# DanielBrosch/SDPSymmetryReduction.jl

Measured on AMD Instinct MI355X. Metric: N x N SDP reductions/sec (admissible_subspace+blockDiagonalize) at N=4096, higher is better.
Workload: dtype int8 square (int32 acc) + f64 eigen

## Files before the change

### sdpsymmetryreduction.jl_amd/csrc/kernels_blockdiag.hip

```cpp
#include <cstdlib>
#include <type_traits>
#include "host_internal.h"
#include "kernel_util.h"

namespace sdpsr {

typedef double v4d __attribute__((ext_vector_type(4)));

__global__ void block_norms_kernel(int64_t n, int64_t ld, const double* __restrict__ M,
                                   const int32_t* __restrict__ space_of, int neig,
                                   unsigned long long* __restrict__ norms) {
    const int64_t len = n * n;
    const int64_t stride = (int64_t)gridDim.x * blockDim.x;
    for (int64_t e0 = (int64_t)blockIdx.x * blockDim.x; e0 < len; e0 += stride) {
        const int64_t e = e0 + threadIdx.x;
        bool valid = e < len;
        int64_t j = valid ? e / n : 0, i = valid ? e - j * n : 0;
        int bi = space_of[i], bj = space_of[j];
        unsigned long long v = valid ? (unsigned long long)__double_as_longlong(fabs(M[i + j * ld])) : 0ull;
        int key = bi * neig + bj;
        int prev_key = __shfl_up(key, 1, 64);
        bool head = ((threadIdx.x & 63) == 0) || prev_key != key;
#pragma unroll
        for (int o = 1; o < 64; o <<= 1) {
// ... 708 lines not shown
    const double* Ti = T + (int64_t)i * n * S1;
    double a0 = 0, a1 = 0;
    if (o < S) {
        const int ca = colA[o], cb = colB[o];
        int r = g;
        for (; r + 64 < n; r += 128) {
            const double qa0 = Qrm[(int64_t)r * S1 + ca], qb0 = Qrm[(int64_t)r * S1 + cb];
            const double ta0 = Ti[(int64_t)r * S1 + ca], tb0 = Ti[(int64_t)r * S1 + cb];
            const double qa1 = Qrm[(int64_t)(r + 64) * S1 + ca], qb1 = Qrm[(int64_t)(r + 64) * S1 + cb];
            const double ta1 = Ti[(int64_t)(r + 64) * S1 + ca], tb1 = Ti[(int64_t)(r + 64) * S1 + cb];
            a0 = fma(qa0, tb0, a0);
            a0 = fma(qb0, ta0, a0);
            a1 = fma(qa1, tb1, a1);
            a1 = fma(qb1, ta1, a1);
        }
        for (; r < n; r += 64) {
            a0 = fma(Qrm[(int64_t)r * S1 + ca], Ti[(int64_t)r * S1 + cb], a0);
            a0 = fma(Qrm[(int64_t)r * S1 + cb], Ti[(int64_t)r * S1 + ca], a0);
        }
    }
    red[threadIdx.x] = a0 + a1;
    __syncthreads();
    if (threadIdx.x < 4 && o < S) {
        double v = 0;
        for (int gg = 0; gg < 64; ++gg) v += red[gg * 4 + threadIdx.x];
        out[(int64_t)i * S + o] = (fabs(v) < atol) ? 0.0 : v;
    }
}

bool basis_image_two_stage_fits(int64_t n, int64_t d, int64_t S1) {
    return n <= 65535 && (2 * (d + 2) * 4 + n * 2) <= 60 * 1024 && d * n * S1 * 8 <= ((int64_t)4 << 30);
}

__global__ void __launch_bounds__(256)
class_sums_small_d_kernel(int n, int d, uint32_t first, int tstride, const uint32_t* __restrict__ L, const double* __restrict__ x,
                          double* __restrict__ out, int64_t ldo) {
    extern __shared__ __attribute__((aligned(16))) double cs_smem[];
    double* sx = cs_smem;
    const int lane = threadIdx.x & 63, wave = threadIdx.x >> 6;
    double* acc = cs_smem + n + (size_t)wave * 64 * tstride;
    double* mine = acc + (size_t)lane * tstride;
    for (int c = threadIdx.x; c < n; c += 256) sx[c] = x[c];
    __syncthreads();
    const int rows_per_round = gridDim.x * 4;
    const int bpr = (n + 511) / 512;
    const int my_rows = (n - blockIdx.x * 4 + rows_per_round - 1) / rows_per_round;
    const int total = my_rows * bpr;
    auto fetch = [&](int bq, uint32_t (&lab)[8]) {
        const int rr = bq / bpr, bb = bq - rr * bpr;
        const int r = blockIdx.x * 4 + rr * rows_per_round + wave;
        const uint32_t* col = L + (int64_t)((bq < total && r < n) ? r : 0) * n;
#pragma unroll
        for (int u = 0; u < 8; ++u) {
            const int c = bb * 512 + u * 64 + lane;
            lab[u] = col[c < n ? c : n - 1];
        }
    };
    auto process = [&](int bq, const uint32_t (&lab)[8]) {
        if (bq >= total) return;
        const int rr = bq / bpr, bb = bq - rr * bpr;
        if (bb == 0)
            for (int i = 0; i <= d; ++i) mine[i] = 0.0;
        double vv[8];
#pragma unroll
        for (int u = 0; u < 8; ++u) {
            const int c = bb * 512 + u * 64 + lane;
            vv[u] = c < n ? sx[c] : 0.0;
        }
#pragma unroll
        for (int u = 0; u < 8; ++u) atomicAdd(&mine[window_label(lab[u], first, (uint32_t)d)], vv[u]);
        if (bb == bpr - 1) {
            const int r = blockIdx.x * 4 + rr * rows_per_round + wave;
            __syncthreads();
            if (r < n)
                for (int i = 1 + lane; i <= d; i += 64) {
                    double t = 0;
                    for (int l2 = 0; l2 < 64; ++l2) t += acc[(size_t)l2 * tstride + i];
                    out[(int64_t)(i - 1) * ldo + r] = t;
                }
            __syncthreads();
        }
    };
    uint32_t qa[8], qb[8], qc[8], qd[8];
    fetch(0, qa);
    fetch(1, qb);
    fetch(2, qc);
#pragma unroll 1
    for (int bq = 0; bq < total; bq += 4) {
        fetch(bq + 3, qd);
        process(bq, qa);
        fetch(bq + 4, qa);
        process(bq + 1, qb);
        fetch(bq + 5, qb);
        process(bq + 2, qc);
        fetch(bq + 6, qc);
        process(bq + 3, qd);
    }
}

__device__ __forceinline__ double bi_weight(uint64_t key, int k) {
    return 0.5 + (double)(sdpsr_fmix64(key + 0x9E3779B97F4A7C15ULL * (uint64_t)(k + 1)) >> 11) * (1.0 / 9007199254740992.0);
}

__global__ void bi_signed_sums_kernel(int n, int S1, const double* __restrict__ Qrm, uint64_t key, double2* __restrict__ X, uint32_t* flag) {
    const int r = blockIdx.x * blockDim.x + threadIdx.x;
    if (blockIdx.x == 0)
        for (int k = threadIdx.x; k <= S1; k += blockDim.x) flag[k] = 0u;
    if (r >= n) return;
    double a = 0, b = 0;
    for (int k = 0; k < S1; ++k) {
        const double q = Qrm[(int64_t)r * S1 + k];
        a += q;
        b = fma(bi_weight(key, k), q, b);
    }
    X[r] = make_double2(a, b);
}

__global__ void bi_pair_vector_kernel(int n, int S1, const double* __restrict__ Qrm, int k1, int k2, double2* __restrict__ X) {
    const int r = blockIdx.x * blockDim.x + threadIdx.x;
    if (r < n) X[r] = make_double2(Qrm[(int64_t)r * S1 + k1], Qrm[(int64_t)r * S1 + k2]);
}

__global__ void __launch_bounds__(256)
bi_contract_pair_kernel(int n, int S1, const double* __restrict__ Qrm, const double2* __restrict__ Y, int k1, int k2, double atol,
                        double* __restrict__ out) {
    __shared__ double red[2][256];
    const int i = blockIdx.x;
    const double2* Yi = Y + (int64_t)i * n;
    double a0 = 0, a1 = 0;
// ... 25 lines not shown
    const int bpr = (n + 511) / 512;
    const int my_rows = (n - (int)blockIdx.x * W + rows_per_round - 1) / rows_per_round;
    const int total = my_rows * bpr;
    auto fetch = [&](int bq, uint32_t (&lab)[8], double2 (&xv)[8]) {
        const int rr = bq / bpr, bb = bq - rr * bpr;
        const int r = blockIdx.x * W + rr * rows_per_round + wave;
        const uint32_t* col = L + (int64_t)((bq < total && r < n) ? r : 0) * n;
#pragma unroll
        for (int u = 0; u < 8; ++u) {
            const int c = bb * 512 + u * 64 + lane;
            const int cc = c < n ? c : n - 1;
            lab[u] = col[cc];
            xv[u] = X[cc];
        }
    };
    auto process = [&](int bq, const uint32_t (&lab)[8], const double2 (&xv)[8]) {
        if (bq >= total) return;
        const int rr = bq / bpr, bb = bq - rr * bpr;
        if (bb == 0)
            for (int i = 0; i <= d; ++i) mine[i] = make_double2(0.0, 0.0);
#pragma unroll
        for (int u = 0; u < 8; ++u) {
            const int c = bb * 512 + u * 64 + lane;
            if (c < n) {
                const uint32_t l = WIN ? window_label(lab[u], first, (uint32_t)d) : lab[u];
                double2 t = mine[l];
                t.x += xv[u].x;
                t.y += xv[u].y;
                mine[l] = t;
            }
        }
        if (bb == bpr - 1) {
            const int r = blockIdx.x * W + rr * rows_per_round + wave;
            __syncthreads();
            if (r < n)
                for (int i = 1 + lane; i <= d; i += 64) {
                    double tx = 0, ty = 0;
                    for (int l2 = 0; l2 < 64; ++l2) {
                        const double2 v = acc[(size_t)l2 * tstride + i];
                        tx += v.x;
                        ty += v.y;
                    }
                    out[(int64_t)(i - 1) * n + r] = make_double2(tx, ty);
                }
            __syncthreads();
        }
    };
    uint32_t la[8], lb[8], lc[8];
    double2 xa[8], xb[8], xc[8];
    fetch(0, la, xa);
    fetch(1, lb, xb);
#pragma unroll 1
    for (int bq = 0; bq < total; bq += 3) {
        fetch(bq + 2, lc, xc);
        process(bq, la, xa);
        fetch(bq + 3, la, xa);
        process(bq + 1, lb, xb);
        fetch(bq + 4, lb, xb);
        process(bq + 2, lc, xc);
    }
}

__global__ void __launch_bounds__(256)
bi_contract_check_kernel(int n, int S1, const double* __restrict__ Qrm, const double2* __restrict__ Y, uint64_t key, double atol,
                         double tol, double* __restrict__ out, uint32_t* __restrict__ flag) {
    __shared__ double red[2][256];
    const int i = blockIdx.x;
    const int k = blockIdx.y * 4 + (threadIdx.x & 3);
    const int g = threadIdx.x >> 2;
    const double2* Yi = Y + (int64_t)i * n;
    double a0 = 0, a1 = 0;
    if (k < S1)
        for (int r0 = g; r0 < n; r0 += 64 * 8) {
            double q[8];
            double2 y[8];
#pragma unroll
            for (int x = 0; x < 8; ++x) {
                const int r = r0 + 64 * x;
                const int rc = r < n ? r : g;
                q[x] = r < n ? Qrm[(int64_t)rc * S1 + k] : 0.0;
                y[x] = Yi[rc];
            }
#pragma unroll
            for (int x = 0; x < 8; ++x) {
                a0 = fma(q[x], y[x].x, a0);
                a1 = fma(q[x], y[x].y, a1);
            }
        }
    red[0][threadIdx.x] = a0;
    red[1][threadIdx.x] = a1;
    __syncthreads();
    if (threadIdx.x < 4 && k < S1) {
        double v0 = 0, v1 = 0;
        for (int gg = 0; gg < 64; ++gg) {
            v0 += red[0][gg * 4 + threadIdx.x];
            v1 += red[1][gg * 4 + threadIdx.x];
        }
        if (!(fabs(v0 - v1 / bi_weight(key, k)) <= tol)) {
            if (atomicExch(&flag[1 + k], 1u) == 0u) atomicAdd(&flag[0], 1u);
        }
        out[(int64_t)i * S1 + k] = (fabs(v0) < atol) ? 0.0 : v0;
    }
}

static void launch_class_sums2(hipStream_t s, int W, int g, size_t lds, int64_t n, int64_t d, uint32_t first, bool plain, int tstride, const uint32_t* L,
                               const double2* X, double2* Y) {
    if (plain && first == 1u) {
        if (W == 4) class_sums2_kernel<4, false><<<g, 256, lds, s>>>((int)n, (int)d, first, tstride, L, X, Y);
        else if (W == 2) class_sums2_kernel<2, false><<<g, 128, lds, s>>>((int)n, (int)d, first, tstride, L, X, Y);
        else class_sums2_kernel<1, false><<<g, 64, lds, s>>>((int)n, (int)d, first, tstride, L, X, Y);
    } else {
        if (W == 4) class_sums2_kernel<4, true><<<g, 256, lds, s>>>((int)n, (int)d, first, tstride, L, X, Y);
        else if (W == 2) class_sums2_kernel<2, true><<<g, 128, lds, s>>>((int)n, (int)d, first, tstride, L, X, Y);
        else class_sums2_kernel<1, true><<<g, 64, lds, s>>>((int)n, (int)d, first, tstride, L, X, Y);
    }
}

int launch_class_sums_pair(hipStream_t s, int64_t n, int64_t d, uint32_t first, bool plain, const uint32_t* L, const double* X, double* Y) {
    const int tstride = (int)((d + 1) | 1);
    const size_t per_wave = (size_t)64 * tstride * sizeof(double2);
    int W = 4;
    while (W > 1 && per_wave * W > 150 * 1024) W >>= 1;
    if (per_wave * W > 150 * 1024 || n < 1 || n > 0x7FFFFFFF / 2) return 0;
    int g = (int)((n + W - 1) / W);
    if (g > 256) g = 256;
    launch_class_sums2(s, W, g, per_wave * W, n, d, first, plain, tstride, L, reinterpret_cast<const double2*>(X), reinterpret_cast<double2*>(Y));
    return W;
}

size_t basis_image_commutative_workspace_doubles(int64_t n, int64_t d) { return (size_t)2 * n * (d + 1); }
bool launch_basis_image_commutative(hipStream_t s, int64_t n, int64_t d, uint32_t first, int64_t S1, const uint32_t* L, const double* Qrm, uint64_t key,
                                    double atol, double tol, double* ws, double* out, uint32_t* flag, bool plain) {
    const int tstride = (int)((d + 1) | 1);
    const size_t per_wave = (size_t)64 * tstride * sizeof(double2);
    int W = 4;
    while (W > 1 && per_wave * W > 150 * 1024) W >>= 1;
    if (per_wave * W > 150 * 1024 || n < 1 || n > 0x7FFFFFFF / 2) return false;
    double2* X = reinterpret_cast<double2*>(ws);
    double2* Y = X + n;
// ... 173 lines not shown
    const int tstride = (int)((d + 1) | 1);
    const size_t per_wave = (size_t)64 * tstride * sizeof(double2);
    int W = 4;
    while (W > 1 && per_wave * W > 150 * 1024) W >>= 1;
    if (per_wave * W > 150 * 1024 || n < 1 || n > 0x7FFFFFFF / 2 || nblocks < 1 || nblocks > 65535) return false;
    double2* X0 = reinterpret_cast<double2*>(ws);
    double2* X1 = X0 + n;
    double2* Y0 = X1 + n;
    double2* Y1 = Y0 + (size_t)d * n;
    double* ginv = reinterpret_cast<double*>(Y1 + (size_t)d * n);
    if ((size_t)S1 * BIB_T * 8 > 48 * 1024) return false;
    bib_vectors_kernel<<<(unsigned)((n + 255) / 256), 256, (size_t)S1 * BIB_T * 8, s>>>((int)n, (int)S1, nblocks, blk_col, blk_size, key, only, Qrm, X0, X1, only < 0 ? flag : nullptr, ginv);
    int g = (int)((n + W - 1) / W);
    if (g > 256) g = 256;
    const size_t lds = per_wave * W;
    for (int pass = 0; pass < 2; ++pass) {
        const double2* X = pass ? X1 : X0;
        double2* Y = pass ? Y1 : Y0;
        launch_class_sums2(s, W, g, lds, n, d, first, plain, tstride, L, X, Y);
    }
    dim3 gc((unsigned)d, only >= 0 ? 1u : (unsigned)nblocks);
    bib_contract_kernel<<<gc, 256, 0, s>>>((int)n, (int)S1, S, blk_col, blk_size, blk_off, Qrm, Y0, Y1, ginv, key, only, atol, tol, out, flag);
    return true;
}

bool blockdiag_set_device_attributes() {
    bool ok = true;
    ok &= hipSuccess == hipFuncSetAttribute(reinterpret_cast<const void*>(&class_sums2_kernel<4, false>), hipFuncAttributeMaxDynamicSharedMemorySize, 150 * 1024);
    ok &= hipSuccess == hipFuncSetAttribute(reinterpret_cast<const void*>(&class_sums2_kernel<4, true>), hipFuncAttributeMaxDynamicSharedMemorySize, 150 * 1024);
    ok &= hipSuccess == hipFuncSetAttribute(reinterpret_cast<const void*>(&class_sums2_kernel<2, false>), hipFuncAttributeMaxDynamicSharedMemorySize, 150 * 1024);
    ok &= hipSuccess == hipFuncSetAttribute(reinterpret_cast<const void*>(&class_sums2_kernel<2, true>), hipFuncAttributeMaxDynamicSharedMemorySize, 150 * 1024);
    ok &= hipSuccess == hipFuncSetAttribute(reinterpret_cast<const void*>(&class_sums2_kernel<1, false>), hipFuncAttributeMaxDynamicSharedMemorySize, 150 * 1024);
    ok &= hipSuccess == hipFuncSetAttribute(reinterpret_cast<const void*>(&class_sums2_kernel<1, true>), hipFuncAttributeMaxDynamicSharedMemorySize, 150 * 1024);
    ok &= hipSuccess == hipFuncSetAttribute(reinterpret_cast<const void*>(&class_sums_small_d_kernel),
                        hipFuncAttributeMaxDynamicSharedMemorySize, 150 * 1024);
    ok &= hipSuccess == hipFuncSetAttribute(reinterpret_cast<const void*>(&small_qtaq_block_norms_kernel),
                        hipFuncAttributeMaxDynamicSharedMemorySize, 104 * 1024);
    ok &= hipSuccess == hipFuncSetAttribute(reinterpret_cast<const void*>(&small_cluster_qtaq_block_norms_kernel),
                        hipFuncAttributeMaxDynamicSharedMemorySize, 104 * 1024);
    ok &= hipSuccess == hipFuncSetAttribute(reinterpret_cast<const void*>(&basis_image_outer_mfma_kernel),
                        hipFuncAttributeMaxDynamicSharedMemorySize, 72 * 1024);
    ok &= hipSuccess == hipFuncSetAttribute(reinterpret_cast<const void*>(&basis_image_rows_kernel<1>),
                        hipFuncAttributeMaxDynamicSharedMemorySize, 64 * 1024);
    ok &= hipSuccess == hipFuncSetAttribute(reinterpret_cast<const void*>(&basis_image_rows_kernel<2>),
                        hipFuncAttributeMaxDynamicSharedMemorySize, 64 * 1024);
    return ok;
}

bool class_sums_supports(int64_t n, int64_t d, int64_t ldo) {
    const int tstride = (int)((d + 1) | 1);
    return ldo == n || ((size_t)n + (size_t)4 * 64 * tstride) * sizeof(double) <= 150 * 1024;
}
void launch_class_sums(hipStream_t s, int64_t n, int64_t d, const uint32_t* L, const double* x, double* out, int64_t ldo, uint32_t first) {
    const int tstride = (int)((d + 1) | 1);
    const size_t lds_small = ((size_t)n + (size_t)4 * 64 * tstride) * sizeof(double);
    if (lds_small <= 150 * 1024) {
        int g = (int)((n + 3) / 4);
        if (g > 256) g = 256;
        class_sums_small_d_kernel<<<g, 256, lds_small, s>>>((int)n, (int)d, first, tstride, L, x, out, ldo);
        return;
    }
    const size_t lds = (size_t)2 * (d + 2) * 4 + (size_t)n * 2 + 16;
    basis_image_rows_kernel<1><<<(unsigned)n, 64, lds, s>>>((int)n, (int)d, first, 1, L, x, out, 0);
}

void launch_basis_image_two_stage(hipStream_t s, int64_t n, int64_t d, uint32_t first, int64_t S1, int64_t S,
// ... 202 lines not shown
```

### sdpsymmetryreduction.jl_amd/csrc/kernels_square_check.hip

```cpp
#include "host_internal.h"
#include "sdpsr_hash.h"

namespace sdpsr {

namespace {

constexpr int CHECK_TILE = 64;

__device__ __forceinline__ void check_packed_ij(int n, int64_t e, int& i, int& j) {
    const float t = (float)(2 * n + 1);
    int jj = (int)((t - sqrtf(fmaxf(t * t - 8.0f * (float)e, 0.0f))) * 0.5f);
    jj = jj < 0 ? 0 : (jj > n - 1 ? n - 1 : jj);
    while ((int64_t)jj * n - (int64_t)jj * (jj - 1) / 2 > e) --jj;
    while (jj + 1 < n && (int64_t)(jj + 1) * n - (int64_t)(jj + 1) * jj / 2 <= e) ++jj;
    j = jj;
    i = jj + (int)(e - ((int64_t)jj * n - (int64_t)jj * (jj - 1) / 2));
}
template <typename LT>
__device__ __forceinline__ uint32_t check_label(const LT* __restrict__ Lp, int n, int a, int b) {
    const int hi = a > b ? a : b, lo = a > b ? b : a;
    return (uint32_t)Lp[(int64_t)lo * n - (int64_t)lo * (lo - 1) / 2 + (hi - lo)];
}

template <int T, typename LT>
__global__ void __launch_bounds__(256)
square_check_ref_kernel(int n, int d, const LT* __restrict__ Lp, const uint32_t* __restrict__ first_idx, uint64_t key0, uint64_t key1,
                        int32_t* __restrict__ c) {
    __shared__ uint32_t xt[SQUARE_CHECK_MAX_CLASSES + 1];
    __shared__ int32_t red[4][T];
    const int k = blockIdx.x, g = blockIdx.y;
    const uint64_t key = g ? key1 : key0;
    for (int l = threadIdx.x; l <= SQUARE_CHECK_MAX_CLASSES; l += blockDim.x) xt[l] = (l && l <= d) ? (uint32_t)sdpsr_class_bits(key, (uint32_t)l) : 0u;
    __syncthreads();
    int32_t acc[T];
#pragma unroll
    for (int t = 0; t < T; ++t) acc[t] = 0;
    const int64_t e = (int64_t)first_idx[k];
    if (e < (int64_t)n * (n + 1) / 2) {
        int i, j;
        check_packed_ij(n, e, i, j);
        for (int m = threadIdx.x; m < n; m += blockDim.x) {
            const uint32_t la = check_label(Lp, n, i, m), lb = check_label(Lp, n, m, j);
            const uint32_t xa = la <= (uint32_t)d ? xt[la] : 0u, xb = lb <= (uint32_t)d ? xt[lb] : 0u;
#pragma unroll
            for (int t = 0; t < T; ++t) acc[t] += __mul24(sdpsr_class_i8(xa, t), sdpsr_class_i8(xb, t));
        }
    }
#pragma unroll
    for (int t = 0; t < T; ++t) {
        int v = acc[t];
        for (int o = 32; o > 0; o >>= 1) v += __shfl_down(v, o);
        if ((threadIdx.x & 63) == 0) red[threadIdx.x >> 6][t] = v;
    }
    __syncthreads();
    if (threadIdx.x < T) c[(int64_t)(g * T + threadIdx.x) * d + k] = red[0][threadIdx.x] + red[1][threadIdx.x] + red[2][threadIdx.x] + red[3][threadIdx.x];
}

template <int T>
struct CheckClass {
    uint32_t xbits;
    int32_t c[T];
};

template <int G, int T, bool ROWS>
__device__ __forceinline__ void check_tile_sums(const uint32_t (*tile)[CHECK_TILE + 1], const CheckClass<T> (*cls)[SQUARE_CHECK_MAX_CLASSES + 1],
                                                const uint32_t (*vw)[CHECK_TILE], int d, int32_t* __restrict__ part_x, int64_t* __restrict__ part_c,
                                                int64_t slot, int64_t gt_stride) {
    const int r = threadIdx.x >> 2, p = threadIdx.x & 3;
    int32_t sx[G * T];
    int64_t sc[G * T];
#pragma unroll
    for (int a = 0; a < G * T; ++a) sx[a] = 0, sc[a] = 0;
#pragma unroll
    for (int q = 0; q < 16; ++q) {
        const int k = 16 * p + q;
        uint32_t l = ROWS ? tile[k][r] : tile[r][k];
        l = l <= (uint32_t)d ? l : 0u;
#pragma unroll
        for (int g = 0; g < G; ++g) {
            const int v = (int)vw[g][k];
            const CheckClass<T> rec = cls[g][l];
#pragma unroll
            for (int t = 0; t < T; ++t) {
                sx[g * T + t] += __mul24(sdpsr_class_i8(rec.xbits, t), v);
                sc[g * T + t] += (int64_t)rec.c[t] * (int64_t)v;
            }
        }
    }
// ... 89 lines not shown
        ws = sw[0][r] + sw[1][r] + sw[2][r] + sw[3][r];
        y[(int64_t)gt * npad + i] = ys;
        w[(int64_t)gt * npad + i] = ws;
        const uint64_t key = (gt / T) ? key1 : key0;
        const int64_t v = i < n ? (int64_t)sdpsr_check_vector(sdpsr_check_vector_key(key), (uint32_t)i) : 0;
        const __int128 e = (__int128)ys * (__int128)ys - (__int128)v * (__int128)ws;
        se[r][0] = (uint64_t)(unsigned __int128)e, se[r][1] = (uint64_t)((unsigned __int128)e >> 64);
    }
    __syncthreads();
    if (threadIdx.x == 0) {
        unsigned __int128 tot = 0;
        for (int k = 0; k < CHECK_TILE; ++k) tot += ((unsigned __int128)se[k][1] << 64) | (unsigned __int128)se[k][0];
        esum[((int64_t)gt * nb + blockIdx.x) * 2] = (uint64_t)tot;
        esum[((int64_t)gt * nb + blockIdx.x) * 2 + 1] = (uint64_t)(tot >> 64);
    }
}

__global__ void __launch_bounds__(64)
square_check_verdict_kernel(int nb, int GT, int T, const uint64_t* __restrict__ esum, uint32_t* __restrict__ bits, uint32_t* __restrict__ flag0,
                            uint32_t* __restrict__ flag1) {
    const int gt = threadIdx.x;
    if (gt >= GT) return;
    unsigned __int128 tot = 0;
    for (int b = 0; b < nb; ++b) tot += ((unsigned __int128)esum[((int64_t)gt * nb + b) * 2 + 1] << 64) | (unsigned __int128)esum[((int64_t)gt * nb + b) * 2];
    const bool differs = tot != 0;
    bits[gt] = differs ? 0u : 1u;
    if (differs) (gt / T ? flag1 : flag0)[0] = 1u;
}

template <typename LT>
void square_check_front(hipStream_t s, const SquareCheck& q, const LT* Lp) {
    const int n = (int)q.n, d = (int)q.d, nb = (int)((q.n + CHECK_TILE - 1) / CHECK_TILE);
    const uint64_t k0 = q.key[0], k1 = q.G > 1 ? q.key[1] : 0;
    const dim3 gr((unsigned)d, (unsigned)q.G), gp((unsigned)nb, (unsigned)nb);
    if (q.T == 2) square_check_ref_kernel<2, LT><<<gr, 256, 0, s>>>(n, d, Lp, q.first_idx, k0, k1, q.c);
    else square_check_ref_kernel<4, LT><<<gr, 256, 0, s>>>(n, d, Lp, q.first_idx, k0, k1, q.c);
#define SDPSR_CHECK_PASS_CASE(GG, TT)                                                                                                          \
    if (q.G == GG && q.T == TT) {                                                                                                              \
        if (q.Lfull) square_check_pass_kernel<GG, TT, true, LT><<<gp, 256, 0, s>>>(n, d, Lp, k0, k1, q.c, q.Lfull, q.part_x, q.part_c);        \
        else square_check_pass_kernel<GG, TT, false, LT><<<gp, 256, 0, s>>>(n, d, Lp, k0, k1, q.c, nullptr, q.part_x, q.part_c);               \
    }
    SDPSR_CHECK_PASS_CASE(1, 2)
    SDPSR_CHECK_PASS_CASE(1, 4)
    SDPSR_CHECK_PASS_CASE(2, 2)
    SDPSR_CHECK_PASS_CASE(2, 4)
#undef SDPSR_CHECK_PASS_CASE
}
}

bool square_check_supports(int64_t n, int64_t d, int G, int T) {
    return n >= 1 && n <= SQUARE_CHECK_MAX_ORDER && d >= 1 && d <= SQUARE_CHECK_MAX_CLASSES && (G == 1 || G == 2) && (T == 2 || T == 4);
}
size_t square_check_ws_bytes(int64_t n, int64_t d, int G, int T) {
    SquareCheck q;
    q.n = n, q.d = d, q.G = G, q.T = T;
    return square_check_ws_carve(q, nullptr, 0);
}
size_t square_check_ws_carve(SquareCheck& q, void* ws, size_t gap) {
    const size_t GT = (size_t)q.G * q.T, nb = (size_t)((q.n + CHECK_TILE - 1) / CHECK_TILE), npad = nb * CHECK_TILE;
    size_t off = 0;
    auto take = [&](size_t bytes) {
        off += gap;
        char* p = ws ? (char*)ws + off : nullptr;
        off += (bytes + 15) / 16 * 16;
        return (void*)p;
    };
    q.c = (int32_t*)take(GT * (size_t)q.d * 4);
    q.part_x = (int32_t*)take(GT * nb * npad * 4);
    q.part_c = (int64_t*)take(GT * nb * npad * 8);
// ... 20 lines not shown
```

### sdpsymmetryreduction.jl_amd/csrc/prof/prof.cpp

```cpp
#include <algorithm>
#include <cmath>
#include <complex>
#include <cstdio>
#include <cstdlib>
#include <cstring>
#include <chrono>
#include <functional>
#include <numeric>

#include <rocblas/rocblas.h>
#include <rocsolver/rocsolver.h>

#include "../host_internal.h"
#include "../../../include/sdpsr_prof.h"

using namespace sdpsr;

namespace sdpsr {
void launch_fill_test_sig(hipStream_t s, int64_t len, int64_t nclasses, uint64_t* sig);
void launch_clock_sampler(hipStream_t s, long long* buf, int ns, const unsigned* flag, long long max_ticks, int* count);
void launch_wall_marker(hipStream_t s, long long* out);
bool launch_band_chase(hipStream_t s, int n, int b, double* A, int64_t ld, unsigned* progress, unsigned* abort_flag, double* d, double* e, int max_wgs);
void launch_band_panel_split(hipStream_t s, int64_t m, int b, double* P, int64_t ldp, double* V, int64_t ldv);
}
// ... 601 lines not shown
extern "C" int sdpsr_profile_label_product_pair(sdpsr_ctx* c, int64_t n, int64_t d, int64_t w, int64_t ldw, int64_t ldy, const uint64_t* keys,
                                                const uint32_t* L_host, const double* W_host, double* Y0_inout, double* Y1_inout, int64_t guard,
                                                int32_t* report) {
    CHECK_CTX(c);
    if (!keys || !L_host || !W_host || !Y0_inout || !Y1_inout || !report || n < 1 || n > MK_MAX_N || d < 0 || ldw < n || ldy < n || ldw > MK_MAX_LD ||
        ldy > MK_MAX_LD || w < 1 || w > 64 || guard < 0 || guard > MK_MAX_GUARD)
        return ctx_fail(c, SDPSR_BAD_ARGUMENT, "label_product_pair: bad arguments");
    LabelSpmmForm f;
    if (!label_spmm_pair_select(n, d, (int)w, &f)) return ctx_fail(c, SDPSR_BAD_ARGUMENT, "label_product_pair: shape not supported by the pair launch");
    if (!mk_labels_ok(L_host, (size_t)n * n, d)) return ctx_fail(c, SDPSR_BAD_ARGUMENT, "label_product_pair: a label exceeds d");
    hipStream_t s = c->stream;
    const size_t yn = (size_t)(ldy * w + guard);
    uint32_t* Lb = (uint32_t*)ctx_buf(c, "prof_l", (size_t)n * n * 4);
    const size_t wn = (size_t)ldw * 64;
    double* W = (double*)ctx_buf(c, "prof_mk_a", wn * 8);
    double* Y0 = (double*)ctx_buf(c, "prof_mk_c", yn * 8);
    double* Y1 = (double*)ctx_buf(c, "prof_mk_b", yn * 8);
    double* part = (double*)ctx_buf(c, "cm_part", label_spmm_pair_partial_doubles(n) * 8);
    if (!Lb || !W || !Y0 || !Y1 || !part) return SDPSR_OUT_OF_MEMORY;
    HIP_TRY(c, hipMemcpyAsync(Lb, L_host, (size_t)n * n * 4, hipMemcpyHostToDevice, s));
    HIP_TRY(c, hipMemcpyAsync(W, W_host, wn * 8, hipMemcpyHostToDevice, s));
    HIP_TRY(c, hipMemcpyAsync(Y0, Y0_inout, yn * 8, hipMemcpyHostToDevice, s));
    HIP_TRY(c, hipMemcpyAsync(Y1, Y1_inout, yn * 8, hipMemcpyHostToDevice, s));
    const bool ran = launch_label_spmm_pair(s, n, Lb, keys, d, W, ldw, (int)w, part, Y0, ldy, Y1, ldy);
    HIP_TRY(c, hipMemcpyAsync(Y0_inout, Y0, yn * 8, hipMemcpyDeviceToHost, s));
    HIP_TRY(c, hipMemcpyAsync(Y1_inout, Y1, yn * 8, hipMemcpyDeviceToHost, s));
    HIP_TRY(c, hipStreamSynchronize(s));
    HIP_TRY(c, hipGetLastError());
    if (!ran) return ctx_fail(c, SDPSR_BAD_ARGUMENT, "label_product_pair: shape not supported by the pair launch");
    report[0] = f.mfma, report[1] = f.tile, report[2] = f.z, report[3] = f.cols_per_block;
    return SDPSR_OK;
}

extern "C" int sdpsr_profile_class_sums2(sdpsr_ctx* c, int64_t n, int64_t d, uint32_t first, int plain, const uint32_t* L_host, const double* X_host,
                                         double* Y_inout, int64_t guard, int32_t* report) {
    CHECK_CTX(c);
    if (!L_host || !X_host || !Y_inout || !report || n < 1 || n > MK_MAX_N || d < 1 || d > 4000 || first < 1 || (plain != 0 && plain != 1) ||
        (plain && first != 1) || guard < 0 || guard > MK_MAX_GUARD)
        return ctx_fail(c, SDPSR_BAD_ARGUMENT, "class_sums2: bad arguments");
    if ((size_t)64 * ((d + 1) | 1) * 16 > 150 * 1024) return ctx_fail(c, SDPSR_BAD_ARGUMENT, "class_sums2: no instance for this many classes");
    if (plain && !mk_labels_ok(L_host, (size_t)n * n, d)) return ctx_fail(c, SDPSR_BAD_ARGUMENT, "class_sums2: a label exceeds d");
    hipStream_t s = c->stream;
    const size_t yn = (size_t)(2 * n * d + guard);
    uint32_t* Lb = (uint32_t*)ctx_buf(c, "prof_l", (size_t)n * n * 4);
    double* X = (double*)ctx_buf(c, "prof_mk_a", (size_t)2 * n * 8);
    double* Y = (double*)ctx_buf(c, "prof_mk_c", yn * 8);
    if (!Lb || !X || !Y) return SDPSR_OUT_OF_MEMORY;
    HIP_TRY(c, hipMemcpyAsync(Lb, L_host, (size_t)n * n * 4, hipMemcpyHostToDevice, s));
    HIP_TRY(c, hipMemcpyAsync(X, X_host, (size_t)2 * n * 8, hipMemcpyHostToDevice, s));
    HIP_TRY(c, hipMemcpyAsync(Y, Y_inout, yn * 8, hipMemcpyHostToDevice, s));
    const int W = launch_class_sums_pair(s, n, d, first, plain != 0, Lb, X, Y);
    HIP_TRY(c, hipMemcpyAsync(Y_inout, Y, yn * 8, hipMemcpyDeviceToHost, s));
    HIP_TRY(c, hipStreamSynchronize(s));
    HIP_TRY(c, hipGetLastError());
    if (!W) return ctx_fail(c, SDPSR_BAD_ARGUMENT, "class_sums2: no instance for this many classes");
    report[0] = W;
    return SDPSR_OK;
}

extern "C" int sdpsr_profile_class_sums(sdpsr_ctx* c, int64_t n, int64_t d, int64_t ldo, const uint32_t* L_host, const double* x_host,
                                        double* out_inout, int64_t guard, int32_t* report) {
    CHECK_CTX(c);
    if (!L_host || !x_host || !out_inout || !report || n < 1 || n > MK_MAX_N || d < 1 || d > 4000 || ldo < n || ldo > MK_MAX_LD || guard < 0 ||
        guard > MK_MAX_GUARD)
        return ctx_fail(c, SDPSR_BAD_ARGUMENT, "class_sums: bad arguments");
    if (!mk_labels_ok(L_host, (size_t)n * n, d)) return ctx_fail(c, SDPSR_BAD_ARGUMENT, "class_sums: a label exceeds d");
    const bool table = class_sums_supports(n, d, n + 1);
    report[0] = class_sums_supports(n, d, ldo) ? 1 : 0;
    report[1] = table ? 1 : 0;
    if (!report[0]) return SDPSR_OK;
    if (!table && !basis_image_two_stage_fits(n, d, 1)) return ctx_fail(c, SDPSR_BAD_ARGUMENT, "class_sums: the fallback does not take this shape");
    hipStream_t s = c->stream;
    const size_t on = (size_t)(ldo * d + guard);
    uint32_t* Lb = (uint32_t*)ctx_buf(c, "prof_l", (size_t)n * n * 4);
    double* x = (double*)ctx_buf(c, "prof_mk_a", (size_t)n * 8);
    double* out = (double*)ctx_buf(c, "prof_mk_c", on * 8);
    if (!Lb || !x || !out) return SDPSR_OUT_OF_MEMORY;
    HIP_TRY(c, hipMemcpyAsync(Lb, L_host, (size_t)n * n * 4, hipMemcpyHostToDevice, s));
    HIP_TRY(c, hipMemcpyAsync(x, x_host, (size_t)n * 8, hipMemcpyHostToDevice, s));
    HIP_TRY(c, hipMemcpyAsync(out, out_inout, on * 8, hipMemcpyHostToDevice, s));
    launch_class_sums(s, n, d, Lb, x, out, ldo, 1);
    HIP_TRY(c, hipMemcpyAsync(out_inout, out, on * 8, hipMemcpyDeviceToHost, s));
    HIP_TRY(c, hipStreamSynchronize(s));
    HIP_TRY(c, hipGetLastError());
    return SDPSR_OK;
}

extern "C" int sdpsr_profile_symmetrize(sdpsr_ctx* c, int64_t m, int64_t ld, double* B_inout, int64_t guard) {
    CHECK_CTX(c);
    if (!B_inout || m < 1 || m > 1024 || ld < m || ld > 2048 || guard < 0 || guard > MK_MAX_GUARD) return ctx_fail(c, SDPSR_BAD_ARGUMENT, "symmetrize: bad arguments");
    hipStream_t s = c->stream;
    const size_t bn = (size_t)(ld * m + guard);
    double* B = (double*)ctx_buf(c, "prof_mk_c", bn * 8);
    if (!B) return SDPSR_OUT_OF_MEMORY;
    HIP_TRY(c, hipMemcpyAsync(B, B_inout, bn * 8, hipMemcpyHostToDevice, s));
    launch_symmetrize(s, m, ld, B);
    HIP_TRY(c, hipMemcpyAsync(B_inout, B, bn * 8, hipMemcpyDeviceToHost, s));
    HIP_TRY(c, hipStreamSynchronize(s));
    HIP_TRY(c, hipGetLastError());
    return SDPSR_OK;
}

extern "C" int sdpsr_profile_extract_symmetric(sdpsr_ctx* c, int64_t m, int64_t mp, int64_t lds, const double* src_host, double* dst_inout, int64_t guard) {
    CHECK_CTX(c);
    if (!src_host || !dst_inout || m < 1 || mp < m || mp > 1024 || lds < m || lds > 2048 || guard < 0 || guard > MK_MAX_GUARD)
        return ctx_fail(c, SDPSR_BAD_ARGUMENT, "extract_symmetric: bad arguments");
    hipStream_t s = c->stream;
    const size_t dn = (size_t)(mp * mp + guard);
    double* src = (double*)ctx_buf(c, "prof_mk_a", (size_t)lds * m * 8);
    double* dst = (double*)ctx_buf(c, "prof_mk_c", dn * 8);
// ... 842 lines not shown
```

Before: 2358.

## Pipeline class-sum kernels, add row-resident variant, widen square-check reference kernel

Several changes land together. The class_sums_small_d kernel gets an incremental-index prefetch ring and issues its label prefetch before the x staging. Per-row __syncthreads are replaced by wave-level fences in the class-sum kernels, and a new class_sums2_rows_kernel keeps X and label batches in registers for n up to 4096. Separately, square_check_ref now uses 1024 threads, handles both keys in one block and unrolls its label loads. The aim is to cut block-wide sync stalls, index arithmetic and load latency, at the cost of more register pressure and relying on waves touching only their own LDS regions.

After: 2448, median of 6. 3.8% higher.

```diff
diff --git a/sdpsymmetryreduction.jl_amd/csrc/kernels_blockdiag.hip b/sdpsymmetryreduction.jl_amd/csrc/kernels_blockdiag.hip
--- a/sdpsymmetryreduction.jl_amd/csrc/kernels_blockdiag.hip
+++ b/sdpsymmetryreduction.jl_amd/csrc/kernels_blockdiag.hip
@@ -764,69 +764,82 @@
     return n <= 65535 && (2 * (d + 2) * 4 + n * 2) <= 60 * 1024 && d * n * S1 * 8 <= ((int64_t)4 << 30);
 }
 
+__device__ __forceinline__ void wave_lds_order() {
+    __builtin_amdgcn_fence(__ATOMIC_ACQ_REL, "wavefront");
+    __builtin_amdgcn_wave_barrier();
+}
+
+constexpr int CLASS_SUMS_DEPTH = 3;
+
 __global__ void __launch_bounds__(256)
 class_sums_small_d_kernel(int n, int d, uint32_t first, int tstride, const uint32_t* __restrict__ L, const double* __restrict__ x,
                           double* __restrict__ out, int64_t ldo) {
+    constexpr int D = CLASS_SUMS_DEPTH, NB = D + 1;
     extern __shared__ __attribute__((aligned(16))) double cs_smem[];
     double* sx = cs_smem;
     const int lane = threadIdx.x & 63, wave = threadIdx.x >> 6;
     double* acc = cs_smem + n + (size_t)wave * 64 * tstride;
     double* mine = acc + (size_t)lane * tstride;
-    for (int c = threadIdx.x; c < n; c += 256) sx[c] = x[c];
-    __syncthreads();
     const int rows_per_round = gridDim.x * 4;
     const int bpr = (n + 511) / 512;
     const int my_rows = (n - blockIdx.x * 4 + rows_per_round - 1) / rows_per_round;
     const int total = my_rows * bpr;
-    auto fetch = [&](int bq, uint32_t (&lab)[8]) {
-        const int rr = bq / bpr, bb = bq - rr * bpr;
-        const int r = blockIdx.x * 4 + rr * rows_per_round + wave;
-        const uint32_t* col = L + (int64_t)((bq < total && r < n) ? r : 0) * n;
+    int fq = 0, fb = 0, fr = blockIdx.x * 4 + wave;
+    auto fetch = [&](uint32_t (&lab)[8]) {
+        const uint32_t* col = L + (int64_t)((fq < total && fr < n) ? fr : 0) * n;
 #pragma unroll
         for (int u = 0; u < 8; ++u) {
-            const int c = bb * 512 + u * 64 + lane;
+            const int c = fb * 512 + u * 64 + lane;
             lab[u] = col[c < n ? c : n - 1];
         }
+        ++fq;
+        if (++fb == bpr) fb = 0, fr += rows_per_round;
     };
-    auto process = [&](int bq, const uint32_t (&lab)[8]) {
-        if (bq >= total) return;
-        const int rr = bq / bpr, bb = bq - rr * bpr;
-        if (bb == 0)
+    int pq = 0, pb = 0, pr = blockIdx.x * 4 + wave;
+    auto process = [&](const uint32_t (&lab)[8]) {
+        if (pq >= total) return;
+        if (pb == 0)
             for (int i = 0; i <= d; ++i) mine[i] = 0.0;
         double vv[8];
 #pragma unroll
         for (int u = 0; u < 8; ++u) {
-            const int c = bb * 512 + u * 64 + lane;
+            const int c = pb * 512 + u * 64 + lane;
             vv[u] = c < n ? sx[c] : 0.0;
         }
 #pragma unroll
         for (int u = 0; u < 8; ++u) atomicAdd(&mine[window_label(lab[u], first, (uint32_t)d)], vv[u]);
-        if (bb == bpr - 1) {
-            const int r = blockIdx.x * 4 + rr * rows_per_round + wave;
-            __syncthreads();
-            if (r < n)
+        ++pq;
+        if (++pb == bpr) {
+            wave_lds_order();
+            if (pr < n)
                 for (int i = 1 + lane; i <= d; i += 64) {
                     double t = 0;
                     for (int l2 = 0; l2 < 64; ++l2) t += acc[(size_t)l2 * tstride + i];
-                    out[(int64_t)(i - 1) * ldo + r] = t;
+                    out[(int64_t)(i - 1) * ldo + pr] = t;
                 }
-            __syncthreads();
+            wave_lds_order();
+            pb = 0, pr += rows_per_round;
         }
     };
-    uint32_t qa[8], qb[8], qc[8], qd[8];
-    fetch(0, qa);
-    fetch(1, qb);
-    fetch(2, qc);
+    uint32_t lab[NB][8];
+#pragma unroll
+    for (int k = 0; k < D; ++k) fetch(lab[k]);
+    for (int c0 = threadIdx.x; c0 < n; c0 += 8 * 256) {
+        double v[8];
+#pragma unroll
+        for (int u = 0; u < 8; ++u) v[u] = x[c0 + u * 256 < n ? c0 + u * 256 : n - 1];
+#pragma unroll
+        for (int u = 0; u < 8; ++u)
+            if (c0 + u * 256 < n) sx[c0 + u * 256] = v[u];
+    }
+    __syncthreads();
 #pragma unroll 1
-    for (int bq = 0; bq < total; bq += 4) {
-        fetch(bq + 3, qd);
-        process(bq, qa);
-        fetch(bq + 4, qa);
-        process(bq + 1, qb);
-        fetch(bq + 5, qb);
-        process(bq + 2, qc);
-        fetch(bq + 6, qc);
-        process(bq + 3, qd);
+    for (int bq = 0; bq < total; bq += NB) {
+#pragma unroll
+        for (int k = 0; k < NB; ++k) {
+            fetch(lab[(k + D) % NB]);
+            process(lab[k]);
+        }
     }
 }
 
@@ -918,7 +931,7 @@
         }
         if (bb == bpr - 1) {
             const int r = blockIdx.x * W + rr * rows_per_round + wave;
-            __syncthreads();
+            wave_lds_order();
             if (r < n)
                 for (int i = 1 + lane; i <= d; i += 64) {
                     double tx = 0, ty = 0;
@@ -929,7 +942,7 @@
                     }
                     out[(int64_t)(i - 1) * n + r] = make_double2(tx, ty);
                 }
-            __syncthreads();
+            wave_lds_order();
         }
     };
     uint32_t la[8], lb[8], lc[8];
@@ -947,6 +960,78 @@
     }
 }
 
+constexpr int CLASS_SUMS2_MAX_ROW_BATCHES = 8;
+
+template <int MB, bool WIN>
+__global__ void __launch_bounds__(256)
+class_sums2_rows_kernel(int n, int d, uint32_t first, int tstride, const uint32_t* __restrict__ L, const double2* __restrict__ X,
+                        double2* __restrict__ out) {
+    extern __shared__ __attribute__((aligned(16))) double2 cs2_smem[];
+    const int lane = threadIdx.x & 63, wave = threadIdx.x >> 6;
+    double2* acc = cs2_smem + (size_t)wave * 64 * tstride;
+    double2* mine = acc + (size_t)lane * tstride;
+    const int rows_per_round = gridDim.x * 4;
+    const int r0 = blockIdx.x * 4 + wave;
+    int tail_c[8];
+#pragma unroll
+    for (int u = 0; u < 8; ++u) {
+        const int c = (MB - 1) * 512 + u * 64 + lane;
+        tail_c[u] = c < n ? c : n - 1;
+    }
+    auto fetch = [&](int r, int bb, uint32_t (&lab)[8]) {
+        const uint32_t* col = L + (int64_t)(r < n ? r : 0) * n;
+#pragma unroll
+        for (int u = 0; u < 8; ++u) lab[u] = col[bb < MB - 1 ? bb * 512 + u * 64 + lane : tail_c[u]];
+    };
+    uint32_t lab[MB][8];
+    double2 xv[MB][8];
+#pragma unroll
+    for (int bb = 0; bb < MB; ++bb) fetch(r0, bb, lab[bb]);
+#pragma unroll
+    for (int bb = 0; bb < MB; ++bb) {
+#pragma unroll
+        for (int u = 0; u < 8; ++u) {
+            const int c = bb * 512 + u * 64 + lane;
+            const double2 v = X[c < n ? c : n - 1];
+            xv[bb][u] = c < n ? v : make_double2(0.0, 0.0);
+        }
+    }
+    __builtin_amdgcn_s_waitcnt(0x0F70);
+#pragma unroll 1
+    for (int r = r0; r < n; r += rows_per_round) {
+#pragma unroll
+        for (int bb = 0; bb < MB; ++bb) {
+            double2* slot[8];
+#pragma unroll
+            for (int u = 0; u < 8; ++u) slot[u] = mine + (WIN ? window_label(lab[bb][u], first, (uint32_t)d) : lab[bb][u]);
+            __builtin_amdgcn_sched_barrier(0);
+            fetch(r + rows_per_round, bb, lab[bb]);
+            __builtin_amdgcn_sched_barrier(0);
+            if (bb == 0)
+                for (int i = 0; i <= d; ++i) mine[i] = make_double2(0.0, 0.0);
+#pragma unroll
+            for (int u = 0; u < 8; ++u) {
+                double2 t = *slot[u];
+                t.x += xv[bb][u].x;
+                t.y += xv[bb][u].y;
+                *slot[u] = t;
+            }
+            __builtin_amdgcn_sched_barrier(0);
+        }
+        wave_lds_order();
+        for (int i = 1 + lane; i <= d; i += 64) {
+            double tx = 0, ty = 0;
+            for (int l2 = 0; l2 < 64; ++l2) {
+                const double2 v = acc[(size_t)l2 * tstride + i];
+                tx += v.x;
+                ty += v.y;
+            }
+            out[(int64_t)(i - 1) * n + r] = make_double2(tx, ty);
+        }
+        wave_lds_order();
+    }
+}
+
 __global__ void __launch_bounds__(256)
 bi_contract_check_kernel(int n, int S1, const double* __restrict__ Qrm, const double2* __restrict__ Y, uint64_t key, double atol,
                          double tol, double* __restrict__ out, uint32_t* __restrict__ flag) {
@@ -991,6 +1076,20 @@
 
 static void launch_class_sums2(hipStream_t s, int W, int g, size_t lds, int64_t n, int64_t d, uint32_t first, bool plain, int tstride, const uint32_t* L,
                                const double2* X, double2* Y) {
+    if (W == 4 && n <= (int64_t)512 * CLASS_SUMS2_MAX_ROW_BATCHES) {
+        const bool win = !(plain && first == 1u);
+#define SDPSR_CS2_ROWS(MB)                                                                                            \
+    case MB:                                                                                                          \
+        if (win) class_sums2_rows_kernel<MB, true><<<g, 256, lds, s>>>((int)n, (int)d, first, tstride, L, X, Y);      \
+        else class_sums2_rows_kernel<MB, false><<<g, 256, lds, s>>>((int)n, (int)d, first, tstride, L, X, Y);         \
+        break;
+        switch ((int)((n + 511) / 512)) {
+            SDPSR_CS2_ROWS(1) SDPSR_CS2_ROWS(2) SDPSR_CS2_ROWS(3) SDPSR_CS2_ROWS(4) SDPSR_CS2_ROWS(5)
+            SDPSR_CS2_ROWS(6) SDPSR_CS2_ROWS(7) SDPSR_CS2_ROWS(8)
+        }
+#undef SDPSR_CS2_ROWS
+        return;
+    }
     if (plain && first == 1u) {
         if (W == 4) class_sums2_kernel<4, false><<<g, 256, lds, s>>>((int)n, (int)d, first, tstride, L, X, Y);
         else if (W == 2) class_sums2_kernel<2, false><<<g, 128, lds, s>>>((int)n, (int)d, first, tstride, L, X, Y);
@@ -1230,6 +1329,12 @@
     ok &= hipSuccess == hipFuncSetAttribute(reinterpret_cast<const void*>(&class_sums2_kernel<2, true>), hipFuncAttributeMaxDynamicSharedMemorySize, 150 * 1024);
     ok &= hipSuccess == hipFuncSetAttribute(reinterpret_cast<const void*>(&class_sums2_kernel<1, false>), hipFuncAttributeMaxDynamicSharedMemorySize, 150 * 1024);
     ok &= hipSuccess == hipFuncSetAttribute(reinterpret_cast<const void*>(&class_sums2_kernel<1, true>), hipFuncAttributeMaxDynamicSharedMemorySize, 150 * 1024);
+#define SDPSR_CS2_ROWS_ATTR(MB)                                                                                                                                         \
+    ok &= hipSuccess == hipFuncSetAttribute(reinterpret_cast<const void*>(&class_sums2_rows_kernel<MB, false>), hipFuncAttributeMaxDynamicSharedMemorySize, 150 * 1024); \
+    ok &= hipSuccess == hipFuncSetAttribute(reinterpret_cast<const void*>(&class_sums2_rows_kernel<MB, true>), hipFuncAttributeMaxDynamicSharedMemorySize, 150 * 1024);
+    SDPSR_CS2_ROWS_ATTR(1) SDPSR_CS2_ROWS_ATTR(2) SDPSR_CS2_ROWS_ATTR(3) SDPSR_CS2_ROWS_ATTR(4) SDPSR_CS2_ROWS_ATTR(5)
+    SDPSR_CS2_ROWS_ATTR(6) SDPSR_CS2_ROWS_ATTR(7) SDPSR_CS2_ROWS_ATTR(8)
+#undef SDPSR_CS2_ROWS_ATTR
     ok &= hipSuccess == hipFuncSetAttribute(reinterpret_cast<const void*>(&class_sums_small_d_kernel),
                         hipFuncAttributeMaxDynamicSharedMemorySize, 150 * 1024);
     ok &= hipSuccess == hipFuncSetAttribute(reinterpret_cast<const void*>(&small_qtaq_block_norms_kernel),
diff --git a/sdpsymmetryreduction.jl_amd/csrc/kernels_square_check.hip b/sdpsymmetryreduction.jl_amd/csrc/kernels_square_check.hip
--- a/sdpsymmetryreduction.jl_amd/csrc/kernels_square_check.hip
+++ b/sdpsymmetryreduction.jl_amd/csrc/kernels_square_check.hip
@@ -22,38 +22,58 @@
     return (uint32_t)Lp[(int64_t)lo * n - (int64_t)lo * (lo - 1) / 2 + (hi - lo)];
 }
 
+constexpr int CHECK_REF_THREADS = 1024, CHECK_REF_UNROLL = 4;
+
 template <int T, typename LT>
-__global__ void __launch_bounds__(256)
-square_check_ref_kernel(int n, int d, const LT* __restrict__ Lp, const uint32_t* __restrict__ first_idx, uint64_t key0, uint64_t key1,
+__global__ void __launch_bounds__(CHECK_REF_THREADS)
+square_check_ref_kernel(int n, int d, int G, const LT* __restrict__ Lp, const uint32_t* __restrict__ first_idx, uint64_t key0, uint64_t key1,
                         int32_t* __restrict__ c) {
-    __shared__ uint32_t xt[SQUARE_CHECK_MAX_CLASSES + 1];
-    __shared__ int32_t red[4][T];
-    const int k = blockIdx.x, g = blockIdx.y;
-    const uint64_t key = g ? key1 : key0;
-    for (int l = threadIdx.x; l <= SQUARE_CHECK_MAX_CLASSES; l += blockDim.x) xt[l] = (l && l <= d) ? (uint32_t)sdpsr_class_bits(key, (uint32_t)l) : 0u;
-    __syncthreads();
-    int32_t acc[T];
-#pragma unroll
-    for (int t = 0; t < T; ++t) acc[t] = 0;
+    __shared__ uint32_t xt[2][SQUARE_CHECK_MAX_CLASSES + 1];
+    __shared__ int32_t red[CHECK_REF_THREADS / 64][2 * T];
+    const int k = blockIdx.x;
+    for (int l = threadIdx.x; l < 2 * (SQUARE_CHECK_MAX_CLASSES + 1); l += CHECK_REF_THREADS) {
+        const int g = l / (SQUARE_CHECK_MAX_CLASSES + 1), ll = l - g * (SQUARE_CHECK_MAX_CLASSES + 1);
+        xt[g][ll] = (g < G && ll && ll <= d) ? (uint32_t)sdpsr_class_bits(g ? key1 : key0, (uint32_t)ll) : 0u;
+    }
+    __syncthreads();
+    int32_t acc[2 * T];
+#pragma unroll
+    for (int a = 0; a < 2 * T; ++a) acc[a] = 0;
     const int64_t e = (int64_t)first_idx[k];
     if (e < (int64_t)n * (n + 1) / 2) {
         int i, j;
         check_packed_ij(n, e, i, j);
-        for (int m = threadIdx.x; m < n; m += blockDim.x) {
-            const uint32_t la = check_label(Lp, n, i, m), lb = check_label(Lp, n, m, j);
-            const uint32_t xa = la <= (uint32_t)d ? xt[la] : 0u, xb = lb <= (uint32_t)d ? xt[lb] : 0u;
-#pragma unroll
-            for (int t = 0; t < T; ++t) acc[t] += __mul24(sdpsr_class_i8(xa, t), sdpsr_class_i8(xb, t));
-        }
-    }
-#pragma unroll
-    for (int t = 0; t < T; ++t) {
-        int v = acc[t];
+        for (int m0 = threadIdx.x; m0 < n; m0 += CHECK_REF_THREADS * CHECK_REF_UNROLL) {
+            uint32_t la[CHECK_REF_UNROLL], lb[CHECK_REF_UNROLL];
+#pragma unroll
+            for (int q = 0; q < CHECK_REF_UNROLL; ++q) {
+                const int m = m0 + q * CHECK_REF_THREADS, mm = m < n ? m : n - 1;
+                la[q] = check_label(Lp, n, i, mm), lb[q] = check_label(Lp, n, mm, j);
+            }
+#pragma unroll
+            for (int q = 0; q < CHECK_REF_UNROLL; ++q) {
+                if (m0 + q * CHECK_REF_THREADS >= n) continue;
+#pragma unroll
+                for (int g = 0; g < 2; ++g) {
+                    const uint32_t xa = la[q] <= (uint32_t)d ? xt[g][la[q]] : 0u, xb = lb[q] <= (uint32_t)d ? xt[g][lb[q]] : 0u;
+#pragma unroll
+                    for (int t = 0; t < T; ++t) acc[g * T + t] += __mul24(sdpsr_class_i8(xa, t), sdpsr_class_i8(xb, t));
+                }
+            }
+        }
+    }
+#pragma unroll
+    for (int a = 0; a < 2 * T; ++a) {
+        int v = acc[a];
         for (int o = 32; o > 0; o >>= 1) v += __shfl_down(v, o);
-        if ((threadIdx.x & 63) == 0) red[threadIdx.x >> 6][t] = v;
-    }
-    __syncthreads();
-    if (threadIdx.x < T) c[(int64_t)(g * T + threadIdx.x) * d + k] = red[0][threadIdx.x] + red[1][threadIdx.x] + red[2][threadIdx.x] + red[3][threadIdx.x];
+        if ((threadIdx.x & 63) == 0) red[threadIdx.x >> 6][a] = v;
+    }
+    __syncthreads();
+    if ((int)threadIdx.x < G * T) {
+        int32_t v = 0;
+        for (int w = 0; w < CHECK_REF_THREADS / 64; ++w) v += red[w][threadIdx.x];
+        c[(int64_t)threadIdx.x * d + k] = v;
+    }
 }
 
 template <int T>
@@ -209,9 +229,9 @@
 void square_check_front(hipStream_t s, const SquareCheck& q, const LT* Lp) {
     const int n = (int)q.n, d = (int)q.d, nb = (int)((q.n + CHECK_TILE - 1) / CHECK_TILE);
     const uint64_t k0 = q.key[0], k1 = q.G > 1 ? q.key[1] : 0;
-    const dim3 gr((unsigned)d, (unsigned)q.G), gp((unsigned)nb, (unsigned)nb);
-    if (q.T == 2) square_check_ref_kernel<2, LT><<<gr, 256, 0, s>>>(n, d, Lp, q.first_idx, k0, k1, q.c);
-    else square_check_ref_kernel<4, LT><<<gr, 256, 0, s>>>(n, d, Lp, q.first_idx, k0, k1, q.c);
+    const dim3 gp((unsigned)nb, (unsigned)nb);
+    if (q.T == 2) square_check_ref_kernel<2, LT><<<(unsigned)d, CHECK_REF_THREADS, 0, s>>>(n, d, q.G, Lp, q.first_idx, k0, k1, q.c);
+    else square_check_ref_kernel<4, LT><<<(unsigned)d, CHECK_REF_THREADS, 0, s>>>(n, d, q.G, Lp, q.first_idx, k0, k1, q.c);
 #define SDPSR_CHECK_PASS_CASE(GG, TT)                                                                                                          \
     if (q.G == GG && q.T == TT) {                                                                                                              \
         if (q.Lfull) square_check_pass_kernel<GG, TT, true, LT><<<gp, 256, 0, s>>>(n, d, Lp, k0, k1, q.c, q.Lfull, q.part_x, q.part_c);        \
diff --git a/sdpsymmetryreduction.jl_amd/csrc/prof/prof.cpp b/sdpsymmetryreduction.jl_amd/csrc/prof/prof.cpp
--- a/sdpsymmetryreduction.jl_amd/csrc/prof/prof.cpp
+++ b/sdpsymmetryreduction.jl_amd/csrc/prof/prof.cpp
@@ -657,6 +657,13 @@
     return SDPSR_OK;
 }
 
+struct ExactLabels {
+    uint32_t* p = nullptr;
+    ~ExactLabels() {
+        if (p) hipFree(p);
+    }
+};
+
 extern "C" int sdpsr_profile_class_sums2(sdpsr_ctx* c, int64_t n, int64_t d, uint32_t first, int plain, const uint32_t* L_host, const double* X_host,
                                          double* Y_inout, int64_t guard, int32_t* report) {
     CHECK_CTX(c);
@@ -667,10 +674,12 @@
     if (plain && !mk_labels_ok(L_host, (size_t)n * n, d)) return ctx_fail(c, SDPSR_BAD_ARGUMENT, "class_sums2: a label exceeds d");
     hipStream_t s = c->stream;
     const size_t yn = (size_t)(2 * n * d + guard);
-    uint32_t* Lb = (uint32_t*)ctx_buf(c, "prof_l", (size_t)n * n * 4);
+    ExactLabels labels;
+    if (hipMalloc((void**)&labels.p, (size_t)n * n * 4) != hipSuccess) return ctx_fail(c, SDPSR_OUT_OF_MEMORY, "class_sums2: labels");
+    uint32_t* Lb = labels.p;
     double* X = (double*)ctx_buf(c, "prof_mk_a", (size_t)2 * n * 8);
     double* Y = (double*)ctx_buf(c, "prof_mk_c", yn * 8);
-    if (!Lb || !X || !Y) return SDPSR_OUT_OF_MEMORY;
+    if (!X || !Y) return SDPSR_OUT_OF_MEMORY;
     HIP_TRY(c, hipMemcpyAsync(Lb, L_host, (size_t)n * n * 4, hipMemcpyHostToDevice, s));
     HIP_TRY(c, hipMemcpyAsync(X, X_host, (size_t)2 * n * 8, hipMemcpyHostToDevice, s));
     HIP_TRY(c, hipMemcpyAsync(Y, Y_inout, yn * 8, hipMemcpyHostToDevice, s));
@@ -697,10 +706,12 @@
     if (!table && !basis_image_two_stage_fits(n, d, 1)) return ctx_fail(c, SDPSR_BAD_ARGUMENT, "class_sums: the fallback does not take this shape");
     hipStream_t s = c->stream;
     const size_t on = (size_t)(ldo * d + guard);
-    uint32_t* Lb = (uint32_t*)ctx_buf(c, "prof_l", (size_t)n * n * 4);
+    ExactLabels labels;
+    if (hipMalloc((void**)&labels.p, (size_t)n * n * 4) != hipSuccess) return ctx_fail(c, SDPSR_OUT_OF_MEMORY, "class_sums: labels");
+    uint32_t* Lb = labels.p;
     double* x = (double*)ctx_buf(c, "prof_mk_a", (size_t)n * 8);
     double* out = (double*)ctx_buf(c, "prof_mk_c", on * 8);
-    if (!Lb || !x || !out) return SDPSR_OUT_OF_MEMORY;
+    if (!x || !out) return SDPSR_OUT_OF_MEMORY;
     HIP_TRY(c, hipMemcpyAsync(Lb, L_host, (size_t)n * n * 4, hipMemcpyHostToDevice, s));
     HIP_TRY(c, hipMemcpyAsync(x, x_host, (size_t)n * 8, hipMemcpyHostToDevice, s));
     HIP_TRY(c, hipMemcpyAsync(out, out_inout, on * 8, hipMemcpyHostToDevice, s));
```
